# iceonsun/rsock

Hardware: AMD Instinct MI355X
Metric: Mpkt/s + GiB/s device-resident EncHead+MD5 encode/decode at 1/2/4/8 GPU (higher is better)
Workload: dtype u8; 1 GPU; C3: 4194304 packets/GPU, 1400-B payloads, encode (tag = one MD5 compression per packet and lane + EncHead + payload copy) then decode + tag verify + compact, device-resident; packets_per_gpu=4194304, packets_total=4194304, payload_bytes=1400, frame_slot_bytes=1440, zero_pad=16, key=hello135, tag=md5_per_lane, parallelism=shard1 (no collective)

## Files before the change

rsock_amd/csrc/rsk_kernels.hip:

```cpp
#include <hip/hip_runtime.h>

#include <algorithm>
#include <cassert>
#include <cstdio>
#include <cstring>
#include <mutex>
#include <vector>

#include "../../include/rsk_codec.h"
#include "rsk_ctx.h"
#include "rsk_enc_dev.h"

namespace {

using rsk::DeviceGuard;
using rsk::enc_args;
using rsk::enc_grid;
using rsk::enc_path;
using rsk::g_last_error;
using rsk::kTwoPassMinPackets;
using rsk::launch_check;
using rsk::sample_next;
using rsk::sampled_mean;
using rsk::set_error;
// ... 514 lines not shown
            ep = base + fp + os_ext(a, fp, a.pay_len[i - 1]);
        }
        bad = s < ep;
        if (!bad) {
            uint64_t b = (ep - r0 + kOsBlock - 1u) / kOsBlock;
            const uint64_t bend = e > r0 ? (e - r0 + kOsBlock - 1u) / kOsBlock : 0u;
            if (bend > b + kOsMaxGapBlocks || bend > m.bcap) bad = true;
            else
                for (; b < bend; ++b) m.bfirst[b] = (uint32_t)i;
        }
        if (i == a.n - 1u) m.ctl[1] = e > r0 ? (uint32_t)((e - r0 + kOsBlock - 1u) / kOsBlock) : 0u;
    }
    if (__ballot(bad) != 0ull && (threadIdx.x & 63u) == 0u)
        __hip_atomic_store(m.ctl, m.epoch, __ATOMIC_RELAXED, __HIP_MEMORY_SCOPE_AGENT);
}

struct OsFrame {
    uint64_t po;
    uint32_t P, p;
};

struct OsLd {
    uint4 A, B, H0, H1;
    uint32_t sh;
};
__device__ __forceinline__ OsLd os_load(const EncArgs &a, const uint4 *heads, uint64_t nr, const OsFrame &F,
                                        uint32_t t) {
    OsLd L;
    const uint64_t lo = F.po & ~15ull, hi = (F.po + (F.P ? F.P : 1u) - 1u) & ~15ull;
    const int64_t src = (int64_t)F.po + (int64_t)t - RSK_HEAD_SIZE;
    const uint64_t c0 = (uint64_t)(src & ~(int64_t)15);
    L.sh = (uint32_t)(src & 15);
    const int64_t c1 = (int64_t)c0 + 16;
    const uint64_t a0 = (int64_t)c0 < (int64_t)lo ? lo : c0 > hi ? hi : c0;
    const uint64_t a1 = c1 < (int64_t)lo ? lo : (uint64_t)c1 > hi ? hi : (uint64_t)c1;
    L.A = ld16<kStream>(a.payload + a0);
    L.B = ld16<kStream>(a.payload + a1);
    L.H0 = heads[F.p];
    L.H1 = heads[nr + F.p];
    return L;
}
__device__ __forceinline__ uint4 os_compose(const OsFrame &F, const OsLd &L, uint32_t t) {
    const uint32_t flen = RSK_HEAD_SIZE + F.P;
    uint4 v = funnel16_lane(L.A, L.B, L.sh);
    const int lim = (int)flen - (int)t;
    if (lim < 16) v = lim > 0 ? rsk::keep_bytes16(v, lim) : make_uint4(0u, 0u, 0u, 0u);
    if (t < 32u) {
        const uint4 z = make_uint4(0u, 0u, 0u, 0u);
        const uint4 hv = t < 16u ? funnel16_lane(L.H0, L.H1, t) : funnel16_lane(L.H1, z, t - 16u);
        const int nh = 32 - (int)t;
        const uint4 mk = nh >= 16 ? make_uint4(~0u, ~0u, ~0u, ~0u) : rsk::keep_bytes16(make_uint4(~0u, ~0u, ~0u, ~0u), nh);
        v = make_uint4((hv.x & mk.x) | (v.x & ~mk.x), (hv.y & mk.y) | (v.y & ~mk.y), (hv.z & mk.z) | (v.z & ~mk.z),
                       (hv.w & mk.w) | (v.w & ~mk.w));
    }
    return v;
}

struct OsWin {
    uint32_t p0;
    uint64_t s, e, po;
    uint32_t P;
};
__device__ __forceinline__ OsWin os_window(const EncArgs &a, uint32_t p0, uint32_t lane) {
    OsWin W;
    W.p0 = p0;
    const uint64_t pj = (uint64_t)p0 + lane;
    uint64_t fo = 0, po = 0;
    uint32_t P = 0;
    if (pj < a.n) {
        P = a.pay_len[pj];
        fo = a.frame_off[pj];
        po = a.pay_off[pj];
    }
    W.s = pj < a.n ? reinterpret_cast<uintptr_t>(a.frame) + fo : ~0ull;
    W.e = pj < a.n ? W.s + os_ext(a, fo, P) : ~0ull;
    W.po = po;
    W.P = P;
    return W;
}

__device__ __forceinline__ void os_block(const EncArgs &a, const uint4 *heads, uint64_t nr, const OsWin &W,
                                         uint32_t jlo, uint32_t jhi, uint64_t B0, uint32_t lane) {
    constexpr int U = kOsBlock / 1024;
    constexpr int32_t kFar = 1 << 30;
    const int64_t ds = (int64_t)(W.s - B0), de = (int64_t)(W.e - B0);
    const int32_t rs = W.s == ~0ull ? kFar : ds < -kFar ? -kFar : ds > kFar ? kFar : (int32_t)ds;
    const int32_t re = W.e == ~0ull ? kFar : de < -kFar ? -kFar : de > kFar ? kFar : (int32_t)de;
    uint32_t j1[U], j2[U];
#pragma unroll
    for (int u = 0; u < U; ++u) {
        j1[u] = 64u;
        j2[u] = 64u;
    }
    for (uint32_t j = jlo; j <= jhi; ++j) {
        const int32_t sj = (int32_t)rdl((uint32_t)rs, j), ej = (int32_t)rdl((uint32_t)re, j);
#pragma unroll
        for (int u = 0; u < U; ++u) {
            const int32_t q = (int32_t)(1024u * u + 16u * lane);
            if (sj <= q) j1[u] = j;
            else if (sj < q + 16 && ej > sj && j2[u] == 64u) j2[u] = j;
        }
    }
    uint32_t c1[U], uu[U], t1[U];
    OsFrame F1[U];
    uint32_t p2[U];
    OsLd L[U];
    uint4 G[U];
#pragma unroll
    for (int u = 0; u < U; ++u) {
        const int32_t q = (int32_t)(1024u * u + 16u * lane);
        const uint32_t k1 = j1[u] & 63u, k2 = j2[u] & 63u;
        const int32_t s1 = __shfl(rs, (int)k1), e1 = __shfl(re, (int)k1), s2 = __shfl(rs, (int)k2);
        const bool h1 = j1[u] < 64u && e1 > q, h2 = j2[u] < 64u;
        c1[u] = h1 ? (uint32_t)(e1 - q >= 16 ? 16 : e1 - q) : 0u;
        uu[u] = h2 ? (uint32_t)(s2 - q) : 16u;
        t1[u] = h1 ? (uint32_t)(q - s1) : 0u;
        F1[u].po = (uint64_t)(uint32_t)__shfl((int)(uint32_t)W.po, (int)k1) |
                   ((uint64_t)(uint32_t)__shfl((int)(uint32_t)(W.po >> 32), (int)k1) << 32);
        F1[u].P = (uint32_t)__shfl((int)W.P, (int)k1);
        if (!h1) {
            F1[u].po = 0u;
            F1[u].P = 1u;
        }
        F1[u].p = W.p0 + k1;
        p2[u] = W.p0 + k2;
        L[u] = os_load(a, heads, nr, F1[u], t1[u]);
        G[u] = heads[p2[u] < a.n ? p2[u] : 0u];
    }
    uint4 v[U];
#pragma unroll
    for (int u = 0; u < U; ++u) {
        v[u] = os_compose(F1[u], L[u], t1[u]);
        if (uu[u] < 16u) {
            const uint4 z = make_uint4(0u, 0u, 0u, 0u);
            const uint4 hv = funnel16_lane(z, G[u], 16u - uu[u]);
            const uint4 mk = rsk::keep_bytes16(make_uint4(~0u, ~0u, ~0u, ~0u), (int)uu[u]);
            v[u] = make_uint4((v[u].x & mk.x) | (hv.x & ~mk.x), (v[u].y & mk.y) | (hv.y & ~mk.y),
                              (v[u].z & mk.z) | (hv.z & ~mk.z), (v[u].w & mk.w) | (hv.w & ~mk.w));
        }
    }
#pragma unroll
    for (int u = 0; u < U; ++u) {
        uint8_t *d = reinterpret_cast<uint8_t *>(B0 + 1024u * u + 16u * lane);
        if (c1[u] == 16u || (uu[u] < 16u && c1[u] == uu[u])) st16<kStream>(d, v[u]);
        else {
            if (c1[u]) rsk::store_range16(d, v[u], 0u, c1[u]);
            if (uu[u] < 16u) rsk::store_range16(d, v[u], uu[u], 16u);
        }
    }
}

__global__ __launch_bounds__(kBlock) void k_encode_os(EncArgs a, const uint4 *heads, uint64_t nr, const uint32_t *bfirst,
                                                      const uint32_t *ctl, uint32_t epoch) {
    const uint32_t lane = threadIdx.x & 63u;
    const uint32_t w = (uint32_t)__builtin_amdgcn_readfirstlane((int)(threadIdx.x >> 6));
    const uint64_t wid = (uint64_t)blockIdx.x * kWavesPerBlock + w, nw = (uint64_t)gridDim.x * kWavesPerBlock;
    if (__hip_atomic_load(ctl, __ATOMIC_RELAXED, __HIP_MEMORY_SCOPE_AGENT) == epoch) {
        const uint32_t *hr = reinterpret_cast<const uint32_t *>(heads);
        for (uint64_t i0 = wid; i0 < a.n; i0 += nw) {
            CopyK<1> c;
            copyk_issue<1>(a, i0, lane, c);
            if (!c.flen[0]) continue;
            uint32_t Hj[8];
#pragma unroll
            for (int t = 0; t < 8; ++t) Hj[t] = hr[4 * ((t < 4 ? 0 : nr) + i0) + (t & 3)];
            copyk_store<1>(a, c, 0, lane, Hj);
        }
        return;
    }
    const uint64_t nb = ctl[1];
    const uint64_t r0 = (reinterpret_cast<uintptr_t>(a.frame) + a.frame_off[0]) & ~(uint64_t)(kOsBlock - 1u);
    const uint64_t b0 = nb * wid / nw, b1 = nb * (wid + 1u) / nw;
    if (b0 >= b1) return;
    OsWin W = os_window(a, bfirst[b0], lane);
    for (uint64_t b = b0; b < b1; ++b) {
        const uint64_t B0 = r0 + b * kOsBlock, B1 = B0 + kOsBlock;
        for (;;) {
            const uint64_t live = __ballot(W.e > B0);
            const uint64_t past = __ballot(W.s >= B1);
            if (past != 0ull || (W.p0 + 64ull >= a.n)) {
                const uint32_t jlo = live ? (uint32_t)__builtin_ctzll(live) : 64u;
                const uint32_t jhi = past ? (uint32_t)__builtin_ctzll(past) : 64u;
                if (jlo < jhi) os_block(a, heads, nr, W, jlo, jhi - 1u, B0, lane);
                break;
            }
            const uint32_t adv = live ? (uint32_t)__builtin_ctzll(live) : 64u;
            if (adv == 0u) {
                os_block(a, heads, nr, W, 0u, 31u, B0, lane);
                W = os_window(a, W.p0 + 32u, lane);
                continue;
            }
            W = os_window(a, W.p0 + adv, lane);
        }
    }
}

template <int MODE, int PU, int U>
__global__ __launch_bounds__(kBlock) void k_encode(EncArgs a, KeySched ks) {
    __shared__ CopyRec recs[kWavesPerBlock][64];
    __shared__ uint32_t cend[kWavesPerBlock][64];
    stage_tags(ks);
    const uint32_t lane = threadIdx.x & 63u, w = threadIdx.x >> 6;
    uint64_t i;
    if (!set_packet((uint64_t)blockIdx.x * kWavesPerBlock + w, lane, a.n, i)) return;
    encode_set<MODE, PU, U>(a, ks, i, lane, recs[w], cend[w]);
}

struct Dec {
    uint32_t hlen, cmd, id0, id1, conv;
    uint64_t key;
    uint32_t poff, plen;
    int32_t st;
};

template <bool SLOT>
__device__ __forceinline__ Dec decode_frame_t(const uint8_t *base, int nread, bool close,
                                              const KeySched &ks) {
    Dec o = {0, 0, 0, 0, 0, 0, 0, 0, RSK_RECV_DROP};
    if (nread > RSK_HEAD_SIZE) {
        uint32_t w[8];
        if (SLOT || (reinterpret_cast<uintptr_t>(base) & 15u) == 0) {
            const uint4 A = reinterpret_cast<const uint4 *>(base)[0];
            const uint4 B = reinterpret_cast<const uint4 *>(base)[1];
            w[0] = A.x; w[1] = A.y; w[2] = A.z; w[3] = A.w;
            w[4] = B.x; w[5] = B.y; w[6] = B.z; w[7] = B.w;
        } else {
            rsk::load_window16<8>(base, base + nread - 1, w);
        }
        const uint32_t len = w[2] & 0xffu;
        const int dl = nread - 8 - (int)len;
        if ((int)len <= nread - 8 && dl > 0) {
            const uint32_t b = (SLOT || len == (uint32_t)RSK_ENC_HEAD_SIZE) ? (w[7] >> 24) : base[8 + len];
            uint32_t t0, t1;
            tag_of<true>(ks, b, t0, t1);
            if (t0 == w[0] && t1 == w[1]) {
                o.st = RSK_RECV_VALID;
                o.hlen = len;
                o.cmd = (w[2] >> 8) & 0xffu;
                o.id0 = (w[2] >> 16) | (w[3] << 16);
                o.id1 = (w[3] >> 16) | (w[4] << 16);
                o.conv = (w[4] >> 16) | (w[5] << 16);
                o.key = (uint64_t)((w[5] >> 16) | (w[6] << 16)) |
                        ((uint64_t)((w[6] >> 16) | (w[7] << 16)) << 32);
                o.poff = 8u + len;
                o.plen = (uint32_t)dl;
            }
        }
    } else if (close) {
        o.st = RSK_RECV_CLOSE;
    }
    return o;
}

__device__ __forceinline__ Dec decode_frame(const uint8_t *base, int nread, bool close, const KeySched &ks) {
    return decode_frame_t<false>(base, nread, close, ks);
}

struct DecOut {
    uint8_t *hlen, *cmd, *id;
    uint32_t *conv;
    uint64_t *key;
    uint16_t *pay_off, *pay_len;
    int8_t *status;
    uint64_t *masks;
};

__device__ __forceinline__ void store_dec(const DecOut &d, uint64_t i, const Dec &o) {
    d.hlen[i] = (uint8_t)o.hlen;
    d.cmd[i] = (uint8_t)o.cmd;
    *reinterpret_cast<uint2 *>(d.id + 8 * i) = make_uint2(o.id0, o.id1);
    d.conv[i] = o.conv;
    d.key[i] = o.key;
    d.pay_off[i] = (uint16_t)o.poff;
    d.pay_len[i] = (uint16_t)o.plen;
    d.status[i] = (int8_t)o.st;
}

constexpr unsigned long long kCmpIncl = 1ull << 32;
constexpr unsigned long long kCmpTaint = 1ull << 33;
constexpr int kCmpEpochShift = 34;
constexpr uint32_t kCmpEpochMod = 0x3fffffffu;
constexpr uint32_t kCmpSpinMax = 1u << 22;

__device__ __forceinline__ unsigned long long cmp_wait(unsigned long long *s, uint32_t epoch, bool &timed_out) {
    unsigned long long v;
    uint32_t spins = 0;
    do {
        v = __hip_atomic_load(s, __ATOMIC_RELAXED, __HIP_MEMORY_SCOPE_AGENT);
    } while ((uint32_t)(v >> kCmpEpochShift) != epoch && ++spins < kCmpSpinMax);
    if ((uint32_t)(v >> kCmpEpochShift) == epoch) return v;
    timed_out = true;
    return kCmpIncl;
}

__device__ __forceinline__ bool cmp_wait_incl_clean(unsigned long long *s, uint32_t epoch) {
    unsigned long long v;
    uint32_t spins = 0;
    do {
        v = __hip_atomic_load(s, __ATOMIC_RELAXED, __HIP_MEMORY_SCOPE_AGENT);
    } while (((uint32_t)(v >> kCmpEpochShift) != epoch || !(v & kCmpIncl)) && ++spins < kCmpSpinMax);
    return (uint32_t)(v >> kCmpEpochShift) == epoch && (v & kCmpIncl) && !(v & kCmpTaint);
}

__device__ uint32_t cmp_lookback(unsigned long long *st, uint32_t b, uint32_t agg, uint32_t lane, uint32_t epoch,
                                 bool &to) {
    const unsigned long long tag = (unsigned long long)epoch << kCmpEpochShift;
    if (b == 0u) {
        if (lane == 0u) __hip_atomic_store(st, tag | kCmpIncl | agg, __ATOMIC_RELAXED, __HIP_MEMORY_SCOPE_AGENT);
        return 0u;
    }
    if (lane == 0u) __hip_atomic_store(st + b, tag | agg, __ATOMIC_RELAXED, __HIP_MEMORY_SCOPE_AGENT);
    uint32_t excl = 0;
    for (int64_t top = (int64_t)b - 1;; top -= 64) {
        const int64_t j = top - (int64_t)lane;
        bool lto = false;
        const unsigned long long v = j >= 0 ? cmp_wait(st + j, epoch, lto) : kCmpIncl;
        if (__ballot(lto)) to = true;
        const uint64_t im = __ballot((v & kCmpIncl) != 0ull);
        uint32_t val = (uint32_t)v;
        if (im && lane > (uint32_t)__builtin_ctzll(im)) val = 0u;
#pragma unroll
        for (int off = 32; off; off >>= 1) val += __shfl_xor(val, off);
        excl += val;
        if (im) break;
    }
    if (lane == 0u)
        __hip_atomic_store(st + b, tag | kCmpIncl | (to ? kCmpTaint : 0ull) | (excl + agg), __ATOMIC_RELAXED,
                           __HIP_MEMORY_SCOPE_AGENT);
    return excl;
}

__device__ __forceinline__ void compact_epilogue(const DecOut &d, bool valid, uint64_t i) {
    const uint64_t m = __ballot(valid);
    if ((threadIdx.x & 63u) == 0u) d.masks[i >> 6] = m;
}

struct DecArgs {
    const uint8_t *frame;
    const uint64_t *frame_off;
    const uint16_t *frame_len;
    const uint8_t *close;
    uint32_t n;
};

__global__ __launch_bounds__(kBlock) void k_decode(DecArgs a, DecOut d, KeySched ks) {
    stage_tags(ks);
    const uint64_t i = (uint64_t)blockIdx.x * kBlock + threadIdx.x;
    bool valid = false;
    if (i < a.n) {
        const Dec o = decode_frame(a.frame + a.frame_off[i], (int)a.frame_len[i],
                                   a.close ? a.close[i] != 0 : false, ks);
        store_dec(d, i, o);
        valid = o.st == RSK_RECV_VALID;
    }
    if (d.masks) compact_epilogue(d, valid, i);
}

__global__ __launch_bounds__(kBlock) void k_decode_hdr(DecArgs a, DecOut d, KeySched ks) {
    stage_tags(ks);
    const uint64_t i = (uint64_t)blockIdx.x * kBlock + threadIdx.x;
    bool valid = false;
    if (i < a.n) {
        const Dec o = decode_frame_t<true>(a.frame + 32u * i, (int)a.frame_len[i], a.close ? a.close[i] != 0 : false,
                                           ks);
        store_dec(d, i, o);
        valid = o.st == RSK_RECV_VALID;
    }
    if (d.masks) compact_epilogue(d, valid, i);
}

struct EncHdrArgs {
    const uint8_t *b0;
    const uint16_t *pay_len;
    const uint8_t *cmd;
    const uint32_t *conv;
    const uint64_t *conn_key;
    const uint8_t *id;
    uint8_t *hdr;
    int32_t *status;
    uint32_t id_lo, id_hi, n;
};

__global__ __launch_bounds__(kBlock) void k_encode_hdr(EncHdrArgs a, KeySched ks) {
    stage_tags(ks);
    const uint64_t i = (uint64_t)blockIdx.x * kBlock + threadIdx.x;
    if (i >= a.n) return;
    const uint32_t P = a.pay_len[i];
    const int32_t st = P == 0 ? RSK_SEND_RESET : (P > RSK_MAX_PAYLOAD ? RSK_SEND_OVERSIZE : (int32_t)(RSK_HEAD_SIZE + P));
    uint32_t H[8] = {0, 0, 0, 0, 0, 0, 0, 0};
    if (st > 0) {
        const uint32_t b0 = a.b0[i];
        tag_of(ks, b0, H[0], H[1]);
        uint32_t id0 = a.id_lo, id1 = a.id_hi;
        if (a.id) {
            const uint2 v = *reinterpret_cast<const uint2 *>(a.id + 8 * i);
            id0 = v.x;
            id1 = v.y;
        }
        head_words(a.cmd[i], id0, id1, a.conv[i], a.conn_key[i], b0, H);
    }
    st16<0>(a.hdr + 32u * i, make_uint4(H[0], H[1], H[2], H[3]));
    st16<0>(a.hdr + 32u * i + 16u, make_uint4(H[4], H[5], H[6], H[7]));
    a.status[i] = st;
}

struct ParseArgs {
    const uint8_t *cap;
    const uint64_t *cap_off;
    const uint32_t *wire_len;
    const uint32_t *cap_len;
    uint32_t *src, *dst;
    uint16_t *sp, *dp;
    uint32_t *seq, *ack;
    uint8_t *flag;
    int8_t *pst;
    uint16_t *cpo, *cpl;
    int datalink, flags;
    uint32_t n;
    uint32_t slot;
};

struct ParseRes {
    int ps;
    uint32_t src, dst, sp, dp, seq, ack, fl, payo, plen;
    Dec o;
};

template <int L, bool SLOT, bool HWIN>
__device__ __forceinline__ ParseRes parse_one(const ParseArgs &a, const uint8_t *pkt, uint32_t wl, uint32_t cl,
                                              uint32_t av, uint32_t (&hw)[16], const KeySched &ks) {
    int ps = RSK_PARSE_DROP;
    uint32_t src = 0, dst = 0, sp = 0, dp = 0, seq = 0, ack = 0, fl = 0, payo = 0, plen = 0;
    Dec o = {0, 0, 0, 0, 0, 0, 0, 0, RSK_RECV_DROP};
    do {
        if (wl < 44u) break;
        const uint8_t *last = pkt + (av ? av - 1u : 0u);
        if (cl < (uint32_t)L) { ps = RSK_PARSE_MALFORMED; break; }
        if (!HWIN) rsk::load_window16<16>(pkt, last, hw);
        if (L == 14) {
            if ((hw[3] & 0xffffu) != 0x0008u) break;
        } else {
            if (hw[0] != 2u) break;
        }
        constexpr uint32_t ipo = L;
        if (cl < ipo + 20u) { ps = RSK_PARSE_MALFORMED; break; }
        uint32_t ip[5];
#pragma unroll
        for (int k = 0; k < 5; ++k) ip[k] = rsk::funnel(hw[L / 4 + k + 1], hw[L / 4 + k], L & 3);
        if (((ip[2] >> 8) & 0xffu) != 6u) break;
        const uint32_t ihl = (ip[0] & 15u) * 4u;
        const uint32_t tcpo = ipo + ihl;
        if (cl < tcpo + 20u) { ps = RSK_PARSE_MALFORMED; break; }
        uint32_t th[4];
        if (ihl == 20u) {
            constexpr int T = L + 20;
#pragma unroll
            for (int k = 0; k < 4; ++k) th[k] = rsk::funnel(hw[T / 4 + k + 1], hw[T / 4 + k], T & 3);
        } else {
            if (SLOT && tcpo + 16u > av) { ps = RSK_PARSE_SLOT_SHORT; break; }
            rsk::load_window16<4>(pkt + tcpo, last, th);
        }
        const uint32_t thl = ((th[3] & 0xffu) >> 4) * 4u;
        payo = tcpo + thl;
        const int payload_len = (int)rsk::bswap16(ip[0] >> 16) - (int)(ihl + thl);
        fl = (th[3] >> 8) & 0xffu;
        src = ip[4];
        dst = ip[3];
        sp = rsk::bswap16(th[0] >> 16);
        dp = rsk::bswap16(th[0] & 0xffffu);
        seq = rsk::bswap32(th[1]);
        ack = rsk::bswap32(th[2]);
        if ((fl & RSK_TH_SYN) && (a.flags & RSK_PARSE_HAS_ACK_POOL)) {
            if (a.flags & RSK_PARSE_IS_SERVER) {
                uint32_t t = src; src = dst; dst = t;
                t = sp; sp = dp; dp = t;
                t = seq; seq = ack; ack = t;
            }
            ps = RSK_PARSE_SYN;
            break;
        }
        const bool close = (fl & (RSK_TH_FIN | RSK_TH_RST)) != 0;
        if (payload_len < RSK_HASH_BUF_SIZE + 1 && !close) break;
        if (payload_len < -32) break;
        if (payload_len < 0) { ps = RSK_PARSE_MALFORMED; break; }
        if (payload_len + 32 > RSK_MAX_PKT_SIZE) break;
        if ((uint64_t)payo + (uint64_t)payload_len > cl) { ps = RSK_PARSE_MALFORMED; break; }
        if (SLOT && payload_len > RSK_HEAD_SIZE) {
            if (payo + 32u > av) { ps = RSK_PARSE_SLOT_SHORT; break; }
            const uint32_t len = pkt[payo + 8u];
            if (len != (uint32_t)RSK_ENC_HEAD_SIZE && (int)len < payload_len - 8 && payo + 9u + len > av) {
                ps = RSK_PARSE_SLOT_SHORT;
                break;
            }
        }
        seq += (uint32_t)payload_len;
        plen = (uint32_t)payload_len;
        ps = RSK_PARSE_DELIVER;
        o = decode_frame(pkt + payo, payload_len, close, ks);
    } while (false);
    return ParseRes{ps, src, dst, sp, dp, seq, ack, fl, payo, plen, o};
}

__device__ __forceinline__ bool store_parse(const ParseArgs &a, const DecOut &d, uint64_t i, const ParseRes &r) {
    const bool keep = r.ps == RSK_PARSE_DELIVER || r.ps == RSK_PARSE_SYN;
    a.src[i] = keep ? r.src : 0u;
    a.dst[i] = keep ? r.dst : 0u;
    a.sp[i] = (uint16_t)(keep ? r.sp : 0u);
    a.dp[i] = (uint16_t)(keep ? r.dp : 0u);
    a.seq[i] = keep ? r.seq : 0u;
    a.ack[i] = keep ? r.ack : 0u;
    a.flag[i] = (uint8_t)(keep ? r.fl : 0u);
    a.pst[i] = (int8_t)r.ps;
    a.cpo[i] = (uint16_t)(keep ? r.payo : 0u);
    a.cpl[i] = (uint16_t)r.plen;
    store_dec(d, i, r.o);
    return r.o.st == RSK_RECV_VALID;
}

template <int L, bool SLOT>
__global__ __launch_bounds__(kBlock) void k_parse_decode(ParseArgs a, DecOut d, KeySched ks) {
    stage_tags(ks);
    const uint64_t i = (uint64_t)blockIdx.x * kBlock + threadIdx.x;
    bool valid = false;
    if (i < a.n) {
        const uint8_t *pkt = SLOT ? a.cap + (uint64_t)a.slot * i : a.cap + a.cap_off[i];
        const uint32_t wl = a.wire_len[i], cl = a.cap_len[i];
        const uint32_t av = SLOT ? (cl < a.slot ? cl : a.slot) : cl;
        uint32_t hw[16];
        valid = store_parse(a, d, i, parse_one<L, SLOT, false>(a, pkt, wl, cl, av, hw, ks));
    }
    if (d.masks) compact_epilogue(d, valid, i);
}

struct SyncArgs {
    const uint8_t *rec;
    const uint64_t *rec_off;
    const int32_t *nread;
    uint32_t *src, *dst;
    uint16_t *sp, *dp;
    uint32_t *seq, *ack;
    uint8_t *flag;
    int8_t *pst;
    uint16_t *cpo, *cpl;
    uint32_t n;
};

__global__ __launch_bounds__(kBlock) void k_syncinput_decode(SyncArgs a, DecOut d, KeySched ks) {
    stage_tags(ks);
    const uint64_t i = (uint64_t)blockIdx.x * kBlock + threadIdx.x;
    bool valid = false;
    if (i < a.n) {
        const uint8_t *r = a.rec + a.rec_off[i];
        const int nr = a.nread[i];
        uint32_t w[6] = {0u, 0u, 0u, 0u, 0u, 0u};
        Dec o = {0, 0, 0, 0, 0, 0, 0, 0, RSK_RECV_DROP};
        const bool ok = nr >= RSK_TCPINFO_WIRE_SIZE;
        if (ok) {
            rsk::load_window<6>(r, r + (RSK_TCPINFO_WIRE_SIZE - 1), w);
            w[5] &= 0xffu;
            o = decode_frame(r + RSK_TCPINFO_WIRE_SIZE, nr - RSK_TCPINFO_WIRE_SIZE,
                             (w[5] & (RSK_TH_FIN | RSK_TH_RST)) != 0u, ks);
        }
        a.src[i] = w[0];
        a.dst[i] = w[1];
        a.sp[i] = (uint16_t)(w[2] & 0xffffu);
        a.dp[i] = (uint16_t)(w[2] >> 16);
        a.seq[i] = w[3];
        a.ack[i] = w[4];
        a.flag[i] = (uint8_t)w[5];
        a.pst[i] = (int8_t)(ok ? RSK_PARSE_DELIVER : RSK_PARSE_DROP);
        a.cpo[i] = (uint16_t)(ok ? RSK_TCPINFO_WIRE_SIZE : 0);
        a.cpl[i] = (uint16_t)(ok ? nr - RSK_TCPINFO_WIRE_SIZE : 0);
        store_dec(d, i, o);
        valid = o.st == RSK_RECV_VALID;
    }
    if (d.masks) compact_epilogue(d, valid, i);
}

struct FiltArgs {
    const uint8_t *cap;
    const uint64_t *cap_off;
    const uint32_t *cap_len;
    uint8_t *match;
    uint32_t n;
};

template <int L>
struct FPkt {
    uint32_t cl;
    uint32_t w[16];
    uint32_t t[4];
    int lt;
    __device__ __forceinline__ uint32_t b(int k) const { return (w[k >> 2] >> (8 * (k & 3))) & 0xffu; }
    __device__ __forceinline__ uint32_t tb(int k) const { return (t[k >> 2] >> (8 * (k & 3))) & 0xffu; }
    __device__ __forceinline__ uint32_t ihl4() const { return 4u * (b(L) & 15u); }
};

__device__ __forceinline__ bool is_tus(uint32_t pr) { return pr == 6u || pr == 17u || pr == 132u; }

template <int L>
__device__ __forceinline__ int fp_tcp(const FPkt<L> &k) {
    if (k.lt < 0) return -1;
    if (k.lt == 4) return k.cl < L + 10u ? -1 : (int)(k.b(L + 9) == 6u);
    if (k.lt == 6) {
        if (k.cl < L + 7u) return -1;
        const uint32_t nxt = k.b(L + 6);
        if (nxt == 6u) return 1;
        if (nxt != 44u) return 0;
        return k.cl < L + 41u ? -1 : (int)(k.b(L + 40) == 6u);
    }
    return 0;
}

template <int L, int OFF>
__device__ __forceinline__ int fp_addr(const FPkt<L> &k, uint32_t val) {
    if (k.lt < 0) return -1;
    if (k.lt != 4) return 0;
    if (k.cl < L + OFF + 4u) return -1;
    const uint32_t a = k.b(L + OFF) | (k.b(L + OFF + 1) << 8) | (k.b(L + OFF + 2) << 16) | (k.b(L + OFF + 3) << 24);
    return (int)(a == val);
}

template <int L>
__device__ __forceinline__ int fp_ports(const FPkt<L> &k, const rsk_port_list &pl, uint32_t dir) {
    if (pl.n_single == 0 && pl.n_range == 0) return 1;
    if (k.lt < 0) return -1;
    uint32_t port;
    if (k.lt == 4) {
        if (k.cl < L + 10u) return -1;
        if (!is_tus(k.b(L + 9)) || (((k.b(L + 6) & 0x1fu) << 8) | k.b(L + 7)) != 0u) return 0;
        if (k.cl < L + k.ihl4() + dir + 2u) return -1;
    } else if (k.lt == 6) {
        if (k.cl < L + 7u) return -1;
        if (!is_tus(k.b(L + 6))) return 0;
        if (k.cl < L + 40u + dir + 2u) return -1;
    } else {
        return 0;
    }
    port = dir ? ((k.tb(2) << 8) | k.tb(3)) : ((k.tb(0) << 8) | k.tb(1));
    bool hit = false;
    for (uint32_t q = 0; q < pl.n_single; ++q) hit |= port == pl.single[q];
    for (uint32_t q = 0; q < pl.n_range; ++q) hit |= port >= pl.range[q][0] && port <= pl.range[q][1];
    return (int)hit;
}

template <int L>
__device__ __forceinline__ int fp_syn(const FPkt<L> &k, bool want_set) {
    if (k.lt < 0) return -1;
    if (k.lt != 4) return 0;
    if (k.cl < L + 10u) return -1;
    if (k.b(L + 9) != 6u || (((k.b(L + 6) & 0x1fu) << 8) | k.b(L + 7)) != 0u) return 0;
    if (k.cl < L + k.ihl4() + 14u) return -1;
    const bool syn = (k.tb(13) & 2u) != 0u;
    return (int)(want_set ? syn : !syn);
}

template <int L>
__device__ __forceinline__ int fp_main(const FPkt<L> &k, const rsk_capture_filter &f, bool primed) {
    int r = fp_tcp(k);
    if (r != 1) return r;
    if (f.has_src_ip && (r = fp_addr<L, 12>(k, f.src_ip)) != 1) return r;
    if (f.has_dst_ip && (r = primed ? fp_addr<L, 12>(k, f.dst_ip) : fp_addr<L, 16>(k, f.dst_ip)) != 1) return r;
    if ((r = fp_ports(k, f.src_ports, 0u)) != 1) return r;
    return fp_ports(k, f.dst_ports, primed ? 0u : 2u);
}

template <int L>
__device__ __forceinline__ void filter_load(const uint8_t *p, uint32_t cl, FPkt<L> &k) {
    k.cl = cl;
    const uint8_t *last = p + (cl ? cl - 1u : 0u);
    if (cl) rsk::load_window16<16>(p, last, k.w);
    else
#pragma unroll
        for (int q = 0; q < 16; ++q) k.w[q] = 0;
    if (L == 14) {
        k.lt = cl < 14u ? -1 : ({ const uint32_t et = (k.b(12) << 8) | k.b(13); et == 0x0800u ? 4 : et == 0x86ddu ? 6 : 0; });
    } else {
        k.lt = cl < 4u ? -1 : (k.w[0] == 2u ? 4 : (k.w[0] == 24u || k.w[0] == 28u || k.w[0] == 30u) ? 6 : 0);
    }
    const uint32_t th = L + (k.lt == 6 ? 40u : k.ihl4());
#pragma unroll
    for (int q = 0; q < 4; ++q) k.t[q] = 0;
    if (k.lt > 0 && th < cl) rsk::load_window16<4>(p + th, last, k.t);
}

template <int L>
__device__ __forceinline__ bool filter_eval(const FPkt<L> &k, const rsk_capture_filter &f) {
    int r;
    if (!f.is_server) {
        r = fp_main(k, f, false);
    } else {
        r = fp_syn(k, true);
        if (r == 1) r = fp_main(k, f, true);
        if (r == 0) {
            r = fp_main(k, f, false);
            if (r == 1) r = fp_syn(k, false);
        }
    }
    return r == 1;
}

template <int L>
__global__ __launch_bounds__(kBlock) void k_capture_filter(FiltArgs a, DecOut d, rsk_capture_filter f) {
    const uint64_t i = (uint64_t)blockIdx.x * kBlock + threadIdx.x;
    bool m = false;
    if (i < a.n) {
        FPkt<L> k;
        filter_load<L>(a.cap + a.cap_off[i], a.cap_len[i], k);
        m = filter_eval(k, f);
        a.match[i] = m ? 1 : 0;
    }
    if (d.masks) compact_epilogue(d, m, i);
}

template <int L>
__global__ __launch_bounds__(kBlock) void k_filter_parse_decode(ParseArgs a, DecOut d, KeySched ks, uint8_t *match,
                                                                rsk_capture_filter f) {
    stage_tags(ks);
    const uint64_t i = (uint64_t)blockIdx.x * kBlock + threadIdx.x;
    bool valid = false;
    if (i < a.n) {
        const uint8_t *pkt = a.cap + a.cap_off[i];
        const uint32_t wl = a.wire_len[i], cl = a.cap_len[i];
        FPkt<L> k;
        filter_load<L>(pkt, cl, k);
        const bool m = filter_eval(k, f);
        match[i] = m ? 1 : 0;
        ParseRes r = {RSK_PARSE_DROP, 0, 0, 0, 0, 0, 0, 0, 0, 0, {0, 0, 0, 0, 0, 0, 0, 0, RSK_RECV_DROP}};
        if (m) r = parse_one<L, false, true>(a, pkt, wl, cl, cl, k.w, ks);
        valid = store_parse(a, d, i, r);
    }
    if (d.masks) compact_epilogue(d, valid, i);
}

__global__ __launch_bounds__(kBlock) void k_compact(const uint64_t *masks, uint32_t nw, unsigned long long *st,
                                                    uint32_t *valid_idx, uint32_t *n_valid, uint32_t *err,
                                                    uint32_t stall_tile) {
    __shared__ uint64_t ms[64];
    __shared__ uint32_t mex[64];
    __shared__ uint32_t pre, s_agg, s_epoch, s_to;
    const uint32_t t = threadIdx.x, lane = t & 63u, w = t >> 6;
    const uint64_t mb = (uint64_t)blockIdx.x * 64u;
    const bool last = blockIdx.x == gridDim.x - 1u;
    if (w == 0u) {
        const uint32_t e0 = (uint32_t)__hip_atomic_load(st, __ATOMIC_RELAXED, __HIP_MEMORY_SCOPE_AGENT);
        const uint32_t epoch = e0 % kCmpEpochMod + 1u;
        const uint64_t m = mb + lane < nw ? masks[mb + lane] : 0ull;
        const uint32_t c = (uint32_t)__popcll(m);
        uint32_t inc = c;
#pragma unroll
        for (int off = 1; off < 64; off <<= 1) {
            const uint32_t v = __shfl_up(inc, off);
            if (lane >= (uint32_t)off) inc += v;
        }
        ms[lane] = m;
        mex[lane] = inc - c;
        const uint32_t agg = (uint32_t)__shfl((int)inc, 63);
        bool to = false;
        const uint32_t p = blockIdx.x == stall_tile ? 0u : cmp_lookback(st + 1, blockIdx.x, agg, lane, epoch, to);
        if (lane == 0u) {
            pre = p;
            s_agg = agg;
            s_epoch = epoch;
            s_to = to ? 1u : 0u;
            if (to) __hip_atomic_fetch_or(err, RSK_DEVERR_LOOKBACK, __ATOMIC_RELAXED, __HIP_MEMORY_SCOPE_AGENT);
        }
    }
    __syncthreads();
    if (last && blockIdx.x != stall_tile) {
        bool bad = s_to != 0u;
        for (uint32_t j = t; j + 1u < gridDim.x; j += kBlock)
            if (!cmp_wait_incl_clean(st + 1 + j, s_epoch)) bad = true;
        bad = __syncthreads_or(bad);
        if (t == 0u) {
            if (n_valid) *n_valid = bad ? 0xFFFFFFFFu : pre + s_agg;
            if (bad) __hip_atomic_fetch_or(err, RSK_DEVERR_LOOKBACK, __ATOMIC_RELAXED, __HIP_MEMORY_SCOPE_AGENT);
            __hip_atomic_store(st, (unsigned long long)s_epoch, __ATOMIC_RELAXED, __HIP_MEMORY_SCOPE_AGENT);
        }
    }
    if (!valid_idx) return;
#pragma unroll 4
    for (uint32_t r = 0; r < 16u; ++r) {
        const uint32_t j = 4u * r + w;
        const uint64_t m = ms[j];
        if ((m >> lane) & 1ull)
            valid_idx[pre + mex[j] + (uint32_t)__popcll(m & ((1ull << lane) - 1ull))] = (uint32_t)((mb + j) * 64u + lane);
    }
}

struct TcpRecArgs {
    const uint32_t *src, *dst;
    const uint16_t *sp, *dp;
    const uint32_t *seq, *ack;
    const uint8_t *flag;
    uint8_t *rec;
    uint32_t n;
};

__global__ __launch_bounds__(kBlock) void k_tcpinfo_encode(TcpRecArgs a) {
    __shared__ __attribute__((aligned(16))) uint8_t s[kBlock * RSK_TCPINFO_WIRE_SIZE];
    const uint32_t t = threadIdx.x;
    const uint64_t i = (uint64_t)blockIdx.x * kBlock + t;
    if (i < a.n) {
        uint8_t *r = s + RSK_TCPINFO_WIRE_SIZE * t;
        const uint32_t v32[4] = {a.src[i], a.dst[i], a.seq[i], a.ack[i]};
        const uint32_t v16[2] = {a.sp[i], a.dp[i]};
#pragma unroll
        for (int b = 0; b < 4; ++b) {
            r[0 + b] = (uint8_t)(v32[0] >> (8 * b));
            r[4 + b] = (uint8_t)(v32[1] >> (8 * b));
            r[12 + b] = (uint8_t)(v32[2] >> (8 * b));
            r[16 + b] = (uint8_t)(v32[3] >> (8 * b));
        }
        r[8] = (uint8_t)v16[0];
        r[9] = (uint8_t)(v16[0] >> 8);
        r[10] = (uint8_t)v16[1];
        r[11] = (uint8_t)(v16[1] >> 8);
        r[20] = a.flag[i];
    }
    __syncthreads();
    const uint64_t first = (uint64_t)blockIdx.x * kBlock;
    const uint32_t cnt = (uint32_t)min<uint64_t>(kBlock, a.n - first);
    const uint32_t bytes = cnt * RSK_TCPINFO_WIRE_SIZE;
    uint8_t *out = a.rec + first * RSK_TCPINFO_WIRE_SIZE;
    if ((reinterpret_cast<uintptr_t>(out) & 15u) == 0) {
        for (uint32_t c = t; 16u * c < bytes; c += kBlock) {
            if (16u * c + 16u <= bytes) {
                *reinterpret_cast<uint4 *>(out + 16u * c) = *reinterpret_cast<const uint4 *>(s + 16u * c);
            } else {
                for (uint32_t b = 16u * c; b < bytes; ++b) out[b] = s[b];
            }
        }
    } else {
        for (uint32_t b = t; b < bytes; b += kBlock) out[b] = s[b];
    }
}

}
struct ShimIO {
    uint8_t buf[64];
    int32_t ret;
};
namespace {

__global__ void k_shim(ShimIO *io, int op, int len_arg, KeySched ks) {
    if (threadIdx.x != 0) return;
    uint8_t *b = io->buf;
    if (op == 0) {
        uint32_t t0, t1;
        rsk::md5_tag(ks, b[0], t0, t1);
        for (int k = 0; k < 4; ++k) { b[8 + k] = (uint8_t)(t0 >> (8 * k)); b[12 + k] = (uint8_t)(t1 >> (8 * k)); }
        io->ret = 8;
    } else if (op == 1) {
        uint32_t t0, t1;
        rsk::md5_tag(ks, b[8], t0, t1);
        uint32_t e0 = 0, e1 = 0;
        for (int k = 0; k < 4; ++k) { e0 |= (uint32_t)b[k] << (8 * k); e1 |= (uint32_t)b[4 + k] << (8 * k); }
        io->ret = (t0 == e0 && t1 == e1) ? 1 : 0;
    } else if (op == 2) {
        uint32_t id0 = 0, id1 = 0, conv = 0;
        uint64_t key = 0;
        for (int k = 0; k < 4; ++k) {
            id0 |= (uint32_t)b[1 + k] << (8 * k);
            id1 |= (uint32_t)b[5 + k] << (8 * k);
            conv |= (uint32_t)b[12 + k] << (8 * k);
        }
        for (int k = 0; k < 8; ++k) key |= (uint64_t)b[16 + k] << (8 * k);
        uint32_t H[8];
        head_words(b[0], id0, id1, conv, key, 0u, H);
        for (int q = 0; q < 23; ++q) {
            const int f = 8 + q;
            b[32 + q] = (uint8_t)(H[f >> 2] >> (8 * (f & 3)));
        }
        io->ret = RSK_ENC_HEAD_SIZE;
    } else {
        const uint32_t len = b[0];
        if (len_arg < RSK_ENC_HEAD_SIZE || (int)len > len_arg) {
            io->ret = -1;
            return;
        }
        for (int q = 0; q < 23; ++q) b[32 + q] = b[q];
        io->ret = (int)len;
    }
}

__global__ __launch_bounds__(256) void k_tag_table(KeySched ks, uint2 *tab) {
    uint32_t t0, t1;
    rsk::md5_tag(ks, threadIdx.x, t0, t1);
    tab[threadIdx.x] = make_uint2(t0, t1);
}

__device__ __forceinline__ uint64_t splitmix64_at(uint64_t seed, uint64_t i) {
    uint64_t z = seed + (i + 1u) * 0x9E3779B97F4A7C15ull;
    z = (z ^ (z >> 30)) * 0xBF58476D1CE4E5B9ull;
    z = (z ^ (z >> 27)) * 0x94D049BB133111EBull;
    return z ^ (z >> 31);
}

__global__ __launch_bounds__(kBlock) void k_fill_splitmix(uint8_t *dst, uint64_t nbytes, uint64_t seed) {
    const uint64_t nw = nbytes / 8u;
    const uint64_t stride = (uint64_t)gridDim.x * kBlock;
    for (uint64_t w = (uint64_t)blockIdx.x * kBlock + threadIdx.x; w < nw; w += stride) {
        const uint64_t v = splitmix64_at(seed, w);
        if ((reinterpret_cast<uintptr_t>(dst) & 7u) == 0) {
            reinterpret_cast<uint64_t *>(dst)[w] = v;
        } else {
            for (int b = 0; b < 8; ++b) dst[8 * w + b] = (uint8_t)(v >> (8 * b));
        }
    }
    if (blockIdx.x == 0 && threadIdx.x == 0 && nw * 8u < nbytes) {
        const uint64_t v = splitmix64_at(seed, nw);
        for (uint64_t b = nw * 8u; b < nbytes; ++b) dst[b] = (uint8_t)(v >> (8u * (b - nw * 8u)));
    }
}

void build_sched(const uint8_t *key, uint32_t klen, KeySched &ks) {
    std::memset(&ks, 0, sizeof ks);
    uint32_t st[4] = {0x67452301u, 0xefcdab89u, 0x98badcfeu, 0x10325476u};
    const uint32_t nfull = klen / 64u;
    auto words = [](const uint8_t *p, uint32_t (&m)[16]) {
        for (int w = 0; w < 16; ++w)
            m[w] = (uint32_t)p[4 * w] | ((uint32_t)p[4 * w + 1] << 8) | ((uint32_t)p[4 * w + 2] << 16) |
                   ((uint32_t)p[4 * w + 3] << 24);
    };
    for (uint32_t b = 0; b < nfull; ++b) {
        uint32_t m[16];
        words(key + 64u * b, m);
        rsk::md5_compress(st, m);
    }
    std::memcpy(ks.mid, st, sizeof st);
    uint8_t tail[128];
    std::memset(tail, 0, sizeof tail);
    const uint32_t rem = klen - 64u * nfull;
    if (rem) std::memcpy(tail, key + 64u * nfull, rem);
    tail[rem] = 0;
    tail[rem + 1] = 0x80;
    const bool two = rem + 2u + 8u > 64u;
    const uint32_t tl = two ? 128u : 64u;
    const uint64_t bits = ((uint64_t)klen + 1u) * 8u;
    for (int k = 0; k < 8; ++k) tail[tl - 8 + k] = (uint8_t)(bits >> (8 * k));
    uint32_t m[16];
    words(tail, m);
    std::memcpy(ks.blk, m, sizeof m);
    if (two) {
        words(tail + 64, m);
        std::memcpy(ks.pad, m, sizeof m);
        for (int w = 1; w < 14; ++w) assert(ks.pad[w] == 0u);
    }
    ks.bword = (int32_t)(rem / 4u);
    ks.bshift = (int32_t)(8u * (rem % 4u));
    ks.two_blocks = two ? 1 : 0;
    rsk::md5_prefix_steps(ks.mid, ks.blk, ks.bword, ks.pre);
}

}

thread_local char rsk::g_last_error[256] = "";

namespace {

struct Compact {
    uint64_t *masks = nullptr;
    unsigned long long *st = nullptr;
    uint32_t nw = 0, ntiles = 0;
};

int ensure_compact(rsk_ctx *c, uint32_t n, hipStream_t s, Compact &k) {
    k.nw = (uint32_t)(((n + kBlock - 1ull) / kBlock) * kWavesPerBlock);
    k.ntiles = (k.nw + 63u) / 64u;
    unsigned long long *p = nullptr;
    size_t cap = 0;
    int r = rsk::stream_compact(c, s, 1u + 65ull * k.ntiles, &p, &cap);
    if (r) return r;
    const size_t T = (cap - 1u) / 65u;
    k.st = p;
    k.masks = reinterpret_cast<uint64_t *>(p + 1u + T);
    return RSK_OK;
}

template <class F>
int launch_compacted(rsk_ctx *c, uint32_t n, uint32_t *idx, uint32_t *count, hipStream_t st, const char *what,
                     F launch) {
    const bool compact = idx || count;
    Compact k;
    if (compact) {
        int r = ensure_compact(c, n, st, k);
        if (r) return r;
    }
    launch(k.masks);
    int r = launch_check(what);
    if (r || !compact) return r;
    const uint32_t stall = c->compact_stall_tile.exchange(~0u, std::memory_order_relaxed);
    hipLaunchKernelGGL(k_compact, dim3(k.ntiles), dim3(kBlock), 0, st, k.masks, k.nw, k.st, idx, count, c->err_dev,
                       stall);
    return launch_check("k_compact");
}

bool filter_ports_bad(const rsk_capture_filter *f) {
    for (const rsk_port_list *pl : {&f->src_ports, &f->dst_ports}) {
        if (pl->n_single > RSK_FILTER_MAX_PORTS || pl->n_range > RSK_FILTER_MAX_PORTS) return true;
        for (uint32_t q = 0; q < pl->n_range; ++q)
            if (pl->range[q][0] >= pl->range[q][1]) return true;
    }
    return false;
}

int empty_batch(rsk_ctx *c, uint32_t *n_valid, void *stream) {
    if (!n_valid) return RSK_OK;
    DeviceGuard g(c->device);
    if (!g.ok) return RSK_EDEVICE;
    hipError_t e = hipMemsetAsync(n_valid, 0, sizeof(uint32_t), (hipStream_t)stream);
    if (e != hipSuccess) { set_error("hipMemsetAsync", e); return RSK_EDEVICE; }
    return RSK_OK;
}

bool dec_out_ok(const rsk_decode_out *o) {
    return o && o->hlen && o->cmd && o->id && o->conv && o->conn_key && o->pay_off && o->pay_len &&
           o->status && ((reinterpret_cast<uintptr_t>(o->id) & 7u) == 0);
}

DecOut make_dec_out(const rsk_decode_out *o, uint64_t *masks) {
    DecOut d;
    d.hlen = o->hlen; d.cmd = o->cmd; d.id = o->id; d.conv = o->conv; d.key = o->conn_key;
    d.pay_off = o->pay_off; d.pay_len = o->pay_len; d.status = o->status;
    d.masks = masks;
    return d;
}

bool tcp_out_ok(const rsk_tcpinfo_out *t) {
    return t->src && t->dst && t->sp && t->dp && t->seq && t->ack && t->flag && t->parse_status && t->cap_pay_off &&
           t->cap_pay_len;
}

template <class A>
void fill_tcp_out(A &a, const rsk_tcpinfo_out *t) {
    a.src = t->src; a.dst = t->dst; a.sp = t->sp; a.dp = t->dp; a.seq = t->seq; a.ack = t->ack;
    a.flag = t->flag; a.pst = t->parse_status; a.cpo = t->cap_pay_off; a.cpl = t->cap_pay_len;
}

}

namespace rsk {

bool enc_args(uint32_t n, const rsk_encode_in *in, const rsk_encode_out *out, EncArgs &a) {
    if (!in->payload_arena || !in->pay_off || !in->pay_len || !in->cmd || !in->conv || !in->conn_key ||
        !out->frame_arena || !out->frame_off || !out->status)
        return false;
    if (in->id && (reinterpret_cast<uintptr_t>(in->id) & 7u)) return false;
    a.payload = in->payload_arena; a.pay_off = in->pay_off; a.pay_len = in->pay_len; a.cmd = in->cmd;
    a.conv = in->conv; a.conn_key = in->conn_key; a.id = in->id;
    a.frame = out->frame_arena; a.frame_off = out->frame_off; a.status = out->status;
    std::memcpy(&a.id_lo, in->id_uniform, 4);
    std::memcpy(&a.id_hi, in->id_uniform + 4, 4);
    a.n = n;
    a.pad = (out->flags & RSK_ENC_ZERO_PAD128) ? 7u : (out->flags & RSK_ENC_ZERO_PAD16) ? 4u : 0u;
    return true;
}

unsigned enc_grid(uint64_t n) {
    const uint64_t per_sb = (uint64_t)kSetSbw * 64u, rest = n % per_sb;
    const uint64_t waves = n / per_sb * kSetSbw + std::min<uint64_t>(kSetSbw, (rest + kSetGrp - 1) / kSetGrp);
    return (unsigned)((waves + kWavesPerBlock - 1) / kWavesPerBlock);
}

uint32_t sampled_mean(const rsk_ctx *c) {
    const uint32_t s = c->enc_stat_host ? __atomic_load_n(c->enc_stat_host, __ATOMIC_RELAXED) : 0u;
    return s;
}

int enc_path(rsk_ctx *c, uint32_t n, const uint16_t *pay_len, hipStream_t st, const uint64_t *frame_off,
             uint32_t pad) {
    if (c->enc_path) return c->enc_path;
    if (n >= kTwoPassMinPackets && c->enc_stat_dev && !(sampled_mean(c) & kStatValid) && st != nullptr &&
// ... 574 lines not shown
```

Measured before the change: 1803 Mpkt/s.

## Widen compaction decoupled lookback to use all block waves with batched loads

The decoupled-lookback prefix scan in the compaction kernel now spreads predecessor tile status reads across every wave in the block, with four loads per thread issued up front. Each wave reduces its segment, and segments are combined through shared memory, so a round covers far more predecessor tiles than the earlier single wave of 64. The aim is to shorten lookback latency when predecessors have not yet finished. The cost is extra block-wide barriers per round and more global status traffic.

```diff
diff --git a/rsock_amd/csrc/rsk_kernels.hip b/rsock_amd/csrc/rsk_kernels.hip
--- a/rsock_amd/csrc/rsk_kernels.hip
+++ b/rsock_amd/csrc/rsk_kernels.hip
@@ -840,31 +840,51 @@
     return (uint32_t)(v >> kCmpEpochShift) == epoch && (v & kCmpIncl) && !(v & kCmpTaint);
 }
 
-__device__ uint32_t cmp_lookback(unsigned long long *st, uint32_t b, uint32_t agg, uint32_t lane, uint32_t epoch,
-                                 bool &to) {
-    const unsigned long long tag = (unsigned long long)epoch << kCmpEpochShift;
-    if (b == 0u) {
-        if (lane == 0u) __hip_atomic_store(st, tag | kCmpIncl | agg, __ATOMIC_RELAXED, __HIP_MEMORY_SCOPE_AGENT);
-        return 0u;
-    }
-    if (lane == 0u) __hip_atomic_store(st + b, tag | agg, __ATOMIC_RELAXED, __HIP_MEMORY_SCOPE_AGENT);
+constexpr uint32_t kCmpPer = 4;
+constexpr uint32_t kCmpSegs = kCmpPer * kWavesPerBlock;
+constexpr uint32_t kCmpRound = kCmpPer * kBlock;
+
+__device__ __forceinline__ void cmp_publish(unsigned long long *st, uint32_t b, uint32_t epoch, unsigned long long w) {
+    __hip_atomic_store(st + b, ((unsigned long long)epoch << kCmpEpochShift) | w, __ATOMIC_RELAXED,
+                       __HIP_MEMORY_SCOPE_AGENT);
+}
+
+__device__ uint32_t cmp_lookback(unsigned long long *st, uint32_t b, uint32_t t, uint32_t epoch, bool &to,
+                                 unsigned long long *seg) {
+    const uint32_t lane = t & 63u, w = t >> 6;
     uint32_t excl = 0;
-    for (int64_t top = (int64_t)b - 1;; top -= 64) {
-        const int64_t j = top - (int64_t)lane;
-        bool lto = false;
-        const unsigned long long v = j >= 0 ? cmp_wait(st + j, epoch, lto) : kCmpIncl;
-        if (__ballot(lto)) to = true;
-        const uint64_t im = __ballot((v & kCmpIncl) != 0ull);
-        uint32_t val = (uint32_t)v;
-        if (im && lane > (uint32_t)__builtin_ctzll(im)) val = 0u;
-#pragma unroll
-        for (int off = 32; off; off >>= 1) val += __shfl_xor(val, off);
-        excl += val;
-        if (im) break;
-    }
-    if (lane == 0u)
-        __hip_atomic_store(st + b, tag | kCmpIncl | (to ? kCmpTaint : 0ull) | (excl + agg), __ATOMIC_RELAXED,
-                           __HIP_MEMORY_SCOPE_AGENT);
+    bool lto = false;
+    for (int64_t top = (int64_t)b - 1;; top -= kCmpRound) {
+        unsigned long long v[kCmpPer];
+#pragma unroll
+        for (uint32_t k = 0; k < kCmpPer; ++k) {
+            const int64_t j = top - (int64_t)(t + kBlock * k);
+            v[k] = j >= 0 ? __hip_atomic_load(st + j, __ATOMIC_RELAXED, __HIP_MEMORY_SCOPE_AGENT) : 0ull;
+        }
+#pragma unroll
+        for (uint32_t k = 0; k < kCmpPer; ++k) {
+            const int64_t j = top - (int64_t)(t + kBlock * k);
+            if (j < 0) v[k] = kCmpIncl;
+            else if ((uint32_t)(v[k] >> kCmpEpochShift) != epoch) v[k] = cmp_wait(st + j, epoch, lto);
+            const uint64_t im = __ballot((v[k] & kCmpIncl) != 0ull);
+            uint32_t val = (uint32_t)v[k];
+            if (im && lane > (uint32_t)__builtin_ctzll(im)) val = 0u;
+#pragma unroll
+            for (int off = 32; off; off >>= 1) val += __shfl_xor(val, off);
+            if (lane == 0u) seg[kWavesPerBlock * k + w] = (im ? kCmpIncl : 0ull) | val;
+        }
+        __syncthreads();
+        bool end = false;
+#pragma unroll
+        for (uint32_t s = 0; s < kCmpSegs; ++s) {
+            const unsigned long long sv = seg[s];
+            if (!end) excl += (uint32_t)sv;
+            end = end || (sv & kCmpIncl) != 0ull;
+        }
+        if (end) break;
+        __syncthreads();
+    }
+    to = __syncthreads_or(lto) != 0;
     return excl;
 }
 
@@ -1276,14 +1296,15 @@
                                                     uint32_t stall_tile) {
     __shared__ uint64_t ms[64];
     __shared__ uint32_t mex[64];
-    __shared__ uint32_t pre, s_agg, s_epoch, s_to;
+    __shared__ unsigned long long seg[kCmpSegs];
+    __shared__ uint32_t s_agg, s_epoch;
     const uint32_t t = threadIdx.x, lane = t & 63u, w = t >> 6;
     const uint64_t mb = (uint64_t)blockIdx.x * 64u;
     const bool last = blockIdx.x == gridDim.x - 1u;
+    const bool stalled = blockIdx.x == stall_tile;
     if (w == 0u) {
+        const uint64_t m = mb + lane < nw ? masks[mb + lane] : 0ull;
         const uint32_t e0 = (uint32_t)__hip_atomic_load(st, __ATOMIC_RELAXED, __HIP_MEMORY_SCOPE_AGENT);
-        const uint32_t epoch = e0 % kCmpEpochMod + 1u;
-        const uint64_t m = mb + lane < nw ? masks[mb + lane] : 0ull;
         const uint32_t c = (uint32_t)__popcll(m);
         uint32_t inc = c;
 #pragma unroll
@@ -1294,19 +1315,25 @@
         ms[lane] = m;
         mex[lane] = inc - c;
         const uint32_t agg = (uint32_t)__shfl((int)inc, 63);
-        bool to = false;
-        const uint32_t p = blockIdx.x == stall_tile ? 0u : cmp_lookback(st + 1, blockIdx.x, agg, lane, epoch, to);
+        const uint32_t epoch = e0 % kCmpEpochMod + 1u;
         if (lane == 0u) {
-            pre = p;
             s_agg = agg;
             s_epoch = epoch;
-            s_to = to ? 1u : 0u;
+            if (!stalled) cmp_publish(st + 1, blockIdx.x, epoch, (blockIdx.x == 0u ? kCmpIncl : 0ull) | agg);
+        }
+    }
+    __syncthreads();
+    uint32_t pre = 0;
+    bool to = false;
+    if (blockIdx.x != 0u && !stalled) {
+        pre = cmp_lookback(st + 1, blockIdx.x, t, s_epoch, to, seg);
+        if (t == 0u) {
+            cmp_publish(st + 1, blockIdx.x, s_epoch, kCmpIncl | (to ? kCmpTaint : 0ull) | (pre + s_agg));
             if (to) __hip_atomic_fetch_or(err, RSK_DEVERR_LOOKBACK, __ATOMIC_RELAXED, __HIP_MEMORY_SCOPE_AGENT);
         }
     }
-    __syncthreads();
-    if (last && blockIdx.x != stall_tile) {
-        bool bad = s_to != 0u;
+    if (last && !stalled) {
+        bool bad = to;
         for (uint32_t j = t; j + 1u < gridDim.x; j += kBlock)
             if (!cmp_wait_incl_clean(st + 1 + j, s_epoch)) bad = true;
         bad = __syncthreads_or(bad);
```

Result: no change. 1795 Mpkt/s (-0.4%).
